# Sefaice/LearnRayTracing

Hardware: AMD Instinct MI355X
Metric: Mray/s at 1280×720, 4 spp, 8-bounce; 1/2/4/8-GPU scaling (higher is better)
Workload: dtype f32

## Files before the change

### learnraytracing_amd/csrc/lrt_diag.hip

```cpp
#include "lrt_grid_build.h"
#include "lrt_internal.h"

namespace lrt {

LRT_HD float libm_eval(int kind, float x) {
    if (kind == 6 || kind == 7) {
        float sn, cs;
        libm::sincosf(x, &sn, &cs);
        return kind == 6 ? sn : cs;
    }
    return kind == 0   ? libm::sinf(x)
           : kind == 1 ? libm::cosf(x)
           : kind == 2 ? libm::powf5(x)
           : kind == 3 ? libm::powf(x, 0.416666667f)
           : kind == 4 ? sqrt_rn(x)
                       : rcp_rn(x);
}

__global__ void libm_kernel(int kind, const float* __restrict__ in, float* __restrict__ out, long long n) {
    long long i = (long long)blockIdx.x * blockDim.x + threadIdx.x;
    if (i >= n) return;
    float x = in[i];
    out[i] = libm_eval(kind, x);
}


template <int kAcc>
LRT_DEV void scatter_case(const SceneView& sc, int i, const int* ids, const float* rays, const float* recs,
                          const uint32_t* seeds, float* out, int* ret, int* counted, uint32_t* state,
                          bool coherent = false) {
    const Ray r = make_ray(f3(rays[6 * i], rays[6 * i + 1], rays[6 * i + 2]),
                           f3(rays[6 * i + 3], rays[6 * i + 4], rays[6 * i + 5]));
    Hit rec;
// ... 357 lines not shown
        g.all = (const float4*)up(sph.data(), sizeof(float4) * sph.size());
        need.insert(need.end(), {(void*)g.cells, (void*)g.rsph, (void*)g.rid, (void*)g.bsph, (void*)g.bid, (void*)g.all});
    }
    auto release = [&]() {
        for (void* p : owned) (void)hipFree(p);
    };
    if (std::find(need.begin(), need.end(), nullptr) != need.end()) {
        release();
        return fail(LRT_E_NOMEM, "accel eval: device allocation failed");
    }
    const unsigned blocks = (unsigned)((n + 63) / 64);
    if (accel == 1) accel_probe_kernel<kAccBvh><<<blocks, 64>>>(bv, g, (const float*)d_rays, n, o_ids, o_ts, mode == 2);
    else accel_probe_kernel<kAccGrid><<<blocks, 64>>>(bv, g, (const float*)d_rays, n, o_ids, o_ts, 0);
    hipError_t e = hipGetLastError();
    if (e == hipSuccess) e = hipDeviceSynchronize();
    if (e == hipSuccess) e = hipMemcpy(ids, o_ids, sizeof(int) * (size_t)n, hipMemcpyDeviceToHost);
    if (e == hipSuccess) e = hipMemcpy(ts, o_ts, sizeof(float) * (size_t)n, hipMemcpyDeviceToHost);
    release();
    if (e != hipSuccess) return fail(LRT_E_HIP, std::string("accel eval: ") + hipGetErrorString(e));
    return LRT_OK;
}

int lrt_libm_eval_host(int kind, const float* in, float* out, long long n) {
    if (kind < 0 || kind > 7 || !in || !out || n < 0) return fail(LRT_E_INVALID, "invalid libm eval arguments");
    for (long long i = 0; i < n; ++i)
        out[i] = libm_eval(kind, in[i]);
    return LRT_OK;
}

int lrt_libm_eval_device(int kind, const float* d_in, float* d_out, long long n) {
    if (kind < 0 || kind > 7 || !d_in || !d_out || n < 0) return fail(LRT_E_INVALID, "invalid libm eval arguments");
    if (n == 0) return LRT_OK;
    libm_kernel<<<(unsigned)((n + 255) / 256), 256, 0, nullptr>>>(kind, d_in, d_out, n);
    LRT_HIP(hipGetLastError());
    LRT_HIP(hipDeviceSynchronize());
    return LRT_OK;
}


int lrt_kernel_timing(int on) {
    lrt::g_ktiming_on = on != 0;
    lrt::g_ktiming_used = 0;
    return LRT_OK;
}
int lrt_kernel_times(float* ms, int max_n, int* n) {
    if (!n || (max_n > 0 && !ms)) return lrt::fail(LRT_E_INVALID, "lrt_kernel_times: null output");
    int k = 0;
    for (size_t i = 0; i < lrt::g_ktiming_used && k < max_n; ++i) {
        auto& p = lrt::g_ktiming_ev[i];
        LRT_HIP(hipEventSynchronize(p.b));
        float t = 0.0f;
        LRT_HIP(hipEventElapsedTime(&t, p.a, p.b));
        ms[k++] = t;
    }
// ... 6 lines not shown
```

### learnraytracing_amd/csrc/lrt_internal.h

```cpp
#pragma once
#include <hip/hip_runtime.h>
#include <rccl/rccl.h>
#ifndef LRT_ROCTX
#define LRT_ROCTX 0
#endif
#if LRT_ROCTX
#include <rocprofiler-sdk-roctx/roctx.h>
#endif
#include <math.h>
#include <stdio.h>
#include <string.h>

#include <algorithm>
#include <climits>
#include <cmath>
#include <mutex>
#include <type_traits>
#include <string>
#include <vector>

#include "lrt.h"
#include "lrt_diag.h"
#include "lrt_trace.h"

#define LRT_VERSION_STRING "lrt-mi355x 0.4.0 gfx950"

namespace lrt {

constexpr int kBlock = 64;
constexpr int kBlockWavesX = kBlock == 256 ? 2 : 1;
constexpr int kBlockWavesY = kBlock / 64 / kBlockWavesX;
constexpr int WaveCols(int split) { return split <= 8 ? 8 : 64 / split; }
constexpr int kV0Queues = 16;
constexpr int kCtrStride = 64;

constexpr int kMaxDepthSupported = 64;

constexpr int kWavesPerEU = 4;
constexpr int kPoolSamples = 4096;

struct KernelArgs {
    CameraDev cam;
    const float4* sph;
    const float4* mats;
    const int* lights;
    int count, nlights;
    int width, height;
    int x0, xc, y0, rows;
    int rb, rp, rph;
    int frame0, frames, maxDepth;
    float4* out;
    unsigned long long* rays;
    BvhView bv;
    GridView gv;
    int bvh_stack_offset;
    int grid_lds_offset;
    float4* ovf;
    unsigned long long* wtrace;
    unsigned long long* tiles;
    int ndl;
    float4* feat[6];
    int featMax;
    int regenMin;
    int lateFetch;
    const float* lerp;
    float4* samp;
    float* colbuf;
    int poolSlots;
    int splitFrom;
    int split16;
    const int* perm;
    unsigned* tcost;
// ... 57 lines not shown
        void* d_tmp = nullptr;
        size_t tmp_bytes = 0;
        hipEvent_t ev_rec = nullptr;
        bool rec_done = false;
        int donor = -1;
        std::vector<std::pair<hipStream_t, hipEvent_t>> uses;
        unsigned long long tick = 0;
    };
    struct Scratch {
        hipStream_t s = nullptr;
        void* p = nullptr;
        size_t bytes = 0;
        unsigned long long tick = 0;
        hipEvent_t ev = nullptr;
    };
    static constexpr unsigned long long kScratchIdle = 64;
    static constexpr int kScratchSlots = 8;
    Scratch scratch[kScratchSlots];
    static constexpr int kOrderSlots = 8;
    TileOrder order[kOrderSlots];
    unsigned long long order_tick = 0;
    hipStream_t stream = nullptr;
    int count = 0, nlights = 0;
    float4* d_sph = nullptr;
    float4* d_mats = nullptr;
    int* d_lights = nullptr;
    std::vector<lrt_sphere> spheres;
    std::vector<lrt_material> mats;
    float4* d_bvh_nodes = nullptr;
    float4* d_bvh_lsph = nullptr;
    int* d_bvh_lid = nullptr;
    BvhView bvh{};
    int bvh_on = 0;
    bool bvh_built = false;
    int bvh_stack_levels = kBvhStackLevels;
    uint2* d_grid_cells = nullptr;
    float4* d_grid_rsph = nullptr;
    int* d_grid_rid = nullptr;
    float4* d_grid_bsph = nullptr;
    int* d_grid_bid = nullptr;
    GridView gv{};
    bool grid_pick = false;
    bool grid_ok = false;
    bool grid_built = false;

    float* d_frame = nullptr;
// ... 183 lines not shown
```

### learnraytracing_amd/csrc/lrt_pool.h

```cpp
#pragma once

namespace lrt {

enum : int { kPoolIdle = 0, kPoolTrace = 1, kPoolDone = 2, kPoolEnded = 3 };

template <int kPix>
struct PoolTile {
    static constexpr int X = kPix >= 128 ? 16 : kPix >= 32 ? 8 : kPix >= 8 ? 4 : kPix >= 2 ? 2 : 1;
    static constexpr int Y = kPix / X;
    static_assert(X * Y == kPix && kPix <= 256, "kPix: a power of two up to 256");
};

#if defined(__HIP_DEVICE_COMPILE__)
typedef const __attribute__((address_space(4))) KernelArgs* KArgPtr;
__device__ __forceinline__ KArgPtr opaque_args() {
    KArgPtr p = (KArgPtr)__builtin_amdgcn_kernarg_segment_ptr();
    asm volatile("" : "+s"(p));
    return p;
}
#else
typedef const KernelArgs* KArgPtr;
__device__ __forceinline__ KArgPtr opaque_args() { return nullptr; }
#endif

template <int kAcc, int kW>
__device__ __forceinline__ GridView pool_grid_view(float4* smem) {
    GridView g = opaque_args()->gv;
    {
        float4* b = reinterpret_cast<float4*>(reinterpret_cast<char*>(smem) + opaque_args()->bvh_stack_offset);
        g.bsph = b;
        g.bid = reinterpret_cast<const int*>(b + g.nbig);
    }
    if (kW > 1) {
        char* base = reinterpret_cast<char*>(smem) + opaque_args()->grid_lds_offset;
        const unsigned ncell = (unsigned)(g.nx * g.ny * g.nz), nref = g.cells_refs;
        g.rsph = reinterpret_cast<const float4*>(base);
        g.cells = reinterpret_cast<const uint2*>(base + 16 * nref);
        g.rid = reinterpret_cast<const int*>(base + 16 * nref + 8 * ncell);
    }
    return g;
}

constexpr int kPoolGridWaves = 16;
template <int kW>
constexpr int pool_stack_bytes() { return 64 * kTraceLdsLevels * (kW > 1 ? 14 : 16); }

template <int MAXD, bool kLds, int kAcc, int kPix, int kNS = 0, int kW = 1>
__global__ __launch_bounds__(64 * kW, kWavesPerEU) void pool_kernel(
    const KernelArgs a) {
    static_assert(kNS == 0 || (kLds && !kAcc), "a fixed sphere count is for the LDS linear scan");
    static_assert(kW == 1 || (kAcc == kAccGrid && !kLds), "multi-wave blocks: the grid instance");
    constexpr int kLv = kTraceLdsLevels;
    constexpr bool kPacked = kW > 1;
    extern __shared__ float4 smem[];
    const int lane = kW > 1 ? (int)(threadIdx.x & 63u) : (int)threadIdx.x;
    const int tid = threadIdx.x;
    const int wave = kW > 1 ? (int)(threadIdx.x >> 6) : 0;
    const int wid = (int)blockIdx.x * kW + wave;
    const int nwaves = (int)gridDim.x * kW;
    (void)nwaves;
    double* s_pow = reinterpret_cast<double*>(reinterpret_cast<char*>(smem) + kW * pool_stack_bytes<kW>());
    {
        const libm::PowTables g = libm::pow_tables();
        for (int i = tid; i < 16; i += 64 * kW) {
            s_pow[i] = g.invc[i];
            s_pow[16 + i] = g.logc[i];
        }
        for (int i = tid; i < 32; i += 64 * kW) reinterpret_cast<uint64_t*>(s_pow + 32)[i] = g.exp2[i];
    }
    constexpr int kLutBytes = kAcc ? 0 : kRenormBytes;
    float* s_lut = kAcc ? nullptr : reinterpret_cast<float*>(s_pow + 64);
    if (!kAcc) renorm_lut_fill(s_lut, lane, 64);
    float4* s_sph = reinterpret_cast<float4*>(reinterpret_cast<char*>(smem) + kW * pool_stack_bytes<kW>() +
// ... 147 lines not shown
                const unsigned long long waitM = __ballot(state == kPoolIdle || state == kPoolEnded);
                if (waitM && (__popcll(waitM) >= a.regenMin || __ballot(state == kPoolTrace) == 0)) {
                    if (state == kPoolEnded) {
                        sec_count(sc, kSecFold);
                        F3 T = carry;
                        for (int d = depth - 1; d >= 0; --d) {
                            const float4 s = get(d);
                            const float4 b = sc.mats[3 * __float_as_int(s.w) + 2];
                            T = f3(s.x, s.y, s.z) + f3(b.x, b.y, b.z) * T;
                        }
                        slots[3 * k] = T.x;
                        slots[3 * k + 1] = T.y;
                        slots[3 * k + 2] = T.z;
                        state = kPoolIdle;
                    }
                    const unsigned long long needM = waitM;
                    if (state == kPoolIdle) {
                        k = next + __popcll(needM & below);
                        state = kPoolDone;
                        if (k < N) {
                            const int j = k & ((1 << lgP) - 1), f = fr0 + (k >> lgP);
                            const int lx = tx0 + (j & ((1 << lgW) - 1)), ly = ty0 + (j >> lgW);
                            const KArgPtr pa = opaque_args();
                            if (lx < pa->xc && ly < pa->rows) {
                                sec_count(sc, kSecCamera);
                                const int x = pa->x0 + lx;
                                const int rb = pa->rb;
                                const int y = pa->y0 + (ly / rb) * rb * pa->rp + pa->rph * rb + ly % rb;
                                rng = PixelSeed((uint32_t)x, (uint32_t)y, (uint32_t)f);
                                const float u = ((float)x + RandomFloat01(rng)) * invWidth;
                                const float v = ((float)y + RandomFloat01(rng)) * invHeight;
                                const CameraDev cam = pa->cam;
                                r = GetRay(cam, u, v, rng, sc.rnlut);
                                depth = 0;
                                prevLambert = false;
                                pend = false;
                                state = kPoolTrace;
                            } else {
                                state = kPoolIdle;
                            }
                        }
                    }
                    next += __popcll(needM);
                    if constexpr (kLate) {
                        if (!asked && next >= N && fr0 + roundFrames >= fend) {
                            if (lane == 0) fetched = atomicAdd(ctr, 1ull);
                            asked = true;
                        }
                    }
                }
                const unsigned long long traceM = __ballot(state == kPoolTrace);
                if (traceM == 0) {
                    if (__ballot(state == kPoolIdle || state == kPoolEnded) == 0) break;
                    continue;
                }
// ... 6 lines not shown
                int nid = -1;
                float nt = 0.0f;
                bool shade = false, fin = false;
                F3 leaf = f3(0.0f, 0.0f, 0.0f);
                if (state == kPoolTrace) {
                    sec_count(sc, coherent ? kSecHit0 : kSecHit);
                    ++rays;
                    bool lit = false;
                    const bool hasS = pend && dl.on;
                    if constexpr (kAcc == kAccGrid) {
                        const float4 ls = hasS ? sc.sph[dl.li] : make_float4(0.0f, 0.0f, 0.0f, 0.0f);
                        const GridView gv = pool_grid_view<kAcc, kW>(smem);
                        nid = ClosestHitDualGrid<(kW > 1 ? 1 : 0)>(r.orig, r.dir, hasS, dl.l, dl.li, ls, gv, nt, lit);
                    } else if constexpr (kAcc == kAccBvh) {
                        if (coherent) {
                            nid = ClosestHitBVH(r.orig, r.dir, sc.bv, nt, sc.bstk, sc.bstride, nullptr, true);
                        } else {
                            const float4 ls = hasS ? sc.sph[dl.li] : make_float4(0.0f, 0.0f, 0.0f, 0.0f);
                            nid = ClosestHitDualBVH4(r.orig, r.dir, hasS, dl.l, dl.li, ls, sc.bv, nt, lit, sc.bstk,
                                                     sc.bstride);
                        }
                    } else {
                        int sid;
                        DualClosestHit<kNS>(r.orig, r.dir, hasS, dl.l, sc, nid, nt, sid);
                        lit = hasS && sid == dl.li;
                    }
                    if (pend) {
                        if (lit) put(depth, make_float4(carry.x, carry.y, carry.z, __int_as_float(dl.id)));
                        ++depth;
                        pend = false;
                    }
                    if (nid < 0) {
                        const float t = 0.5f * (r.dir.y + 1.0f);
                        leaf = ((1.0f - t) * f3(1.0f, 1.0f, 1.0f) + t * f3(0.5f, 0.7f, 1.0f)) * 0.3f;
                        fin = true;
                    } else {
                        shade = true;
                    }
                }
                if (shade) {
                    const float4 sp4 = sc.sph[nid];
                    Hit rec;
                    rec.pos = point_at(r, nt);
                    rec.normal = normalize(rec.pos - f3(sp4.x, sp4.y, sp4.z));
                    rec.t = nt;
                    const Material mat = load_material(sc.mats, nid);
                    F3 matE = mat.emissive;
                    fin = true;
                    leaf = matE;
                    if (depth < a.maxDepth) {
                        F3 lightE;
                        dl.on = false;
                        if constexpr (kAcc == kAccGrid) sc.gv = pool_grid_view<kAcc, kW>(smem);
                        const F3 X = ScatterDir<kAcc, kNS>(mat, nid, r, rec, lightE, rays, rng, sc, &dl, coherent);
                        sec_count(sc, kSecPost);
                        const F3 dir = renormalize(normalize(X), sc.rnlut);
                        if ((mat.type != 1) | (dot(dir, rec.normal) > 0.0f)) {
                            if (a.ndl && prevLambert) matE = f3(0.0f, 0.0f, 0.0f);
                            prevLambert = mat.type == 0;
                            const F3 e = matE + lightE;
                            put(depth, make_float4(e.x, e.y, e.z, __int_as_float(nid)));
                            if (dl.on) carry = matE + (lightE + dl.contrib);
                            dl.id = nid;
                            pend = true;
                            r.orig = rec.pos;
                            r.dir = dir;
                            fin = false;
                        }
                    }
                }
                if (fin) {
                    carry = leaf;
                    state = kPoolEnded;
                }
            }
            sec_enter(sc, kSecOther, false);
            __builtin_amdgcn_fence(__ATOMIC_RELEASE, "workgroup");
// ... 16 lines not shown
                        float lf[4];
#pragma unroll
                        for (int u = 0; u < 4; ++u) {
                            const float* const cp = slots + 3 * (((t + u) << lgP) + j);
                            c[u] = f3(cp[0], cp[1], cp[2]);
                            const int f = fr0 + t + u;
                            lf[u] = f < kLerpTable ? lerp[f] : (float)f / (float)(f + 1);
                        }
#pragma unroll
                        for (int u = 0; u < 4; ++u) c3 = c3 * lf[u] + c[u] * (1.0f - lf[u]);
                    }
                    for (; t < nfr; ++t) {
                        const float* const cp = slots + 3 * ((t << lgP) + j);
                        const F3 c = f3(cp[0], cp[1], cp[2]);
                        const int f = fr0 + t;
                        const float lerpFac = f < kLerpTable ? lerp[f] : (float)f / (float)(f + 1);
                        c3 = c3 * lerpFac + f3(c.x, c.y, c.z) * (1.0f - lerpFac);
                    }
                    acc.x = c3.x;
                    acc.y = c3.y;
                    acc.z = c3.z;
                    *mpx = acc;
                    if (frame) {
                        const int rb = pa->rb;
                        const int gy = pa->y0 + (my / rb) * rb * pa->rp + pa->rph * rb + my % rb;
                        frame[(size_t)gy * pa->width + pa->x0 + mx] = acc;
                    }
                }
            }
            __builtin_amdgcn_fence(__ATOMIC_RELEASE, "workgroup");
            __builtin_amdgcn_fence(__ATOMIC_ACQUIRE, "workgroup");
        }
        if (a.tcost && lane == 0) a.tcost[tile] = (unsigned)(__builtin_amdgcn_s_memrealtime() - tt0);
        if constexpr (kLate)
            if (!asked && lane == 0) fetched = atomicAdd(ctr, 1ull);
        const unsigned long long n = __shfl(fetched, 0, 64) + (unsigned long long)bq;
        i = n < (unsigned long long)nq ? (int)n : nq;
    }
#ifdef LRT_EXP_SECSTATS
    sec_enter(sc, kSecOther, false);
    if (lane == 0)
        for (int k = 0; k < kSecN; ++k) {
            unsigned long long* g = sc.secstats + 3 * (k + kSecN * (wid & 15));
            atomicAdd(g, sc.sectime[2 + kSecN + k]);
            atomicAdd(g + 1, sc.sectime[2 + 2 * kSecN + k]);
            atomicAdd(g + 2, sc.sectime[2 + k]);
        }
#endif
// ... 20 lines not shown
```

### learnraytracing_amd/csrc/lrt_pool_launch.h

```cpp
#pragma once
#include "lrt_internal.h"
#include "lrt_pool.h"

namespace lrt {

inline int pool_grid_wpb(const KernelArgs& a, size_t stack_w, size_t shared_b, size_t static_b, size_t* grid_b) {
    const size_t ncell = (size_t)a.gv.nx * a.gv.ny * a.gv.nz, nref = a.gv.cells_refs;
    *grid_b = (16 * nref + 8 * ncell + 4 * nref + 15) / 16 * 16;
    if (!a.gv.on || a.gv.nx == 0) return 1;
    int dev = 0, maxb = 0;
    if (hipGetDevice(&dev) != hipSuccess ||
        hipDeviceGetAttribute(&maxb, hipDeviceAttributeMaxSharedMemoryPerBlock, dev) != hipSuccess)
        return 1;
    return kPoolGridWaves * stack_w + shared_b + *grid_b + static_b <= (size_t)maxb ? kPoolGridWaves : 1;
}

template <int MAXD, int kPix>
int launch_pool(KernelArgs a, bool lds, int xc, int rows, hipStream_t s) {
    constexpr int TX = PoolTile<kPix>::X, TY = PoolTile<kPix>::Y;
    constexpr int kW = kPoolGridWaves;
    const long long ntiles = (long long)((xc + TX - 1) / TX) * ((rows + TY - 1) / TY);
    const int acc = a.gv.on ? kAccGrid : a.bv.on ? kAccBvh : kAccScan;
    const size_t bstk = acc == kAccBvh ? sizeof(unsigned short) * ctx().bvh_stack_levels * 64
                        : acc == kAccGrid ? (sizeof(float4) + sizeof(int)) * (size_t)a.gv.nbig : 0;
// ... 8 lines not shown
                  ? pool_grid_wpb(a, pool_stack_bytes<kW>(), kPowTableBytes + (bstk + 15) / 16 * 16, static_b, &grid_b)
                  : 1;
    if (wpb > 1) {
        static signed char raised[kMaxDevices * 4] = {};
        int dev = 0, maxb = 0;
        signed char* r = hipGetDevice(&dev) == hipSuccess && dev >= 0 && dev < kMaxDevices * 4 ? &raised[dev] : nullptr;
        if (r && *r == 0)
            *r = hipDeviceGetAttribute(&maxb, hipDeviceAttributeMaxSharedMemoryPerBlock, dev) == hipSuccess &&
                         hipFuncSetAttribute((const void*)pool_kernel<MAXD, false, kAccGrid, kPix, 0, kW>,
                                             hipFuncAttributeMaxDynamicSharedMemorySize,
                                             maxb - (int)static_b) == hipSuccess
                     ? 1
                     : -1;
        if (!r || *r < 0) wpb = 1;
    }
    const int lv = kTraceLdsLevels;
    const size_t stack = (wpb > 1 ? (size_t)pool_stack_bytes<kW>() * wpb : (size_t)pool_stack_bytes<1>()) +
                         kPowTableBytes + (acc ? 0 : kRenormBytes);
    const size_t scene = lds ? sizeof(float4) * (4 * (size_t)a.count + (size_t)(a.nlights + 3) / 4 + 1) : 0;
    a.bvh_stack_offset = (int)(stack + scene);
    a.grid_lds_offset = wpb > 1 ? (int)(stack + (bstk + 15) / 16 * 16) : 0;
    const size_t ldsb = wpb > 1 ? stack + (bstk + 15) / 16 * 16 + grid_b : stack + scene + bstk;
    const bool fixed = lds && acc == kAccScan && a.count == kFixedSpheres;
    const void* kern = acc == kAccGrid ? (lds ? (const void*)pool_kernel<MAXD, true, kAccGrid, kPix>
                                          : wpb > 1 ? (const void*)pool_kernel<MAXD, false, kAccGrid, kPix, 0, kW>
                                              : (const void*)pool_kernel<MAXD, false, kAccGrid, kPix>)
                       : acc == kAccBvh ? (lds ? (const void*)pool_kernel<MAXD, true, kAccBvh, kPix>
                                               : (const void*)pool_kernel<MAXD, false, kAccBvh, kPix>)
                       : (fixed ? (const void*)pool_kernel<MAXD, true, kAccScan, kPix, kFixedSpheres>
                          : lds ? (const void*)pool_kernel<MAXD, true, kAccScan, kPix>
                                : (const void*)pool_kernel<MAXD, false, kAccScan, kPix>);
    int per_cu = 0;
    hipError_t e = occupancy(&per_cu, kern, 64 * wpb, ldsb);
    if (e != hipSuccess) return hip_fail(e, "hipOccupancyMaxActiveBlocksPerMultiprocessor");
    if (per_cu < 1) return fail(LRT_E_INVALID, "pool_kernel does not fit on a CU");
    int cus = ctx().num_cus;
    for (const auto& m : ctx().masked_streams)
        if (m.first == s) cus = m.second;
    long long blocks = std::max((long long)per_cu * cus, (long long)kV0Queues);
    if (blocks > ntiles) blocks = ntiles;
    const dim3 grid((unsigned)blocks);
    a.ovf = nullptr;
    a.colbuf = nullptr;
    a.tiles = ctx().d_tiles + (size_t)(ctx().tiles_next++ % kQueueSlots) * kTileSetU64;
    a.regenMin = 16;
    a.lateFetch = ntiles < 6LL * (long long)grid.x * wpb ? 1 : 0;
    a.poolSlots = kPix * std::min(a.frames, kPoolSamples / kPix);
// ... 23 lines not shown
    a.splitFrom = split ? (int)(ntiles - ntiles * a.split16 / 16) : (int)ntiles;
    bool probed = false;
    if (record == 1 && pool_probe_mode() > 0 && (pool_probe_mode() == 2 || !users[1])) {
        Context::TileOrder& o = *users[0];
        KernelArgs pa = a;
        pa.bvh_stack_offset = 0;
        e = launch_tile_probe(pa, acc, o, (int)ntiles, TX, TY, bstk, s);
        if (e != hipSuccess) {
            o.state = 0;
            return hip_fail(e, "tile cost probe");
        }
        a.perm = o.d_perm;
        users[1] = nullptr;
        probed = true;
    }
    kernel_timing(s, 0);
    if (acc == kAccGrid) {
        if (lds) pool_kernel<MAXD, true, kAccGrid, kPix><<<grid, 64, ldsb, s>>>(a);
        else if (wpb > 1) pool_kernel<MAXD, false, kAccGrid, kPix, 0, kW><<<grid, 64 * kW, ldsb, s>>>(a);
        else pool_kernel<MAXD, false, kAccGrid, kPix><<<grid, 64, ldsb, s>>>(a);
    } else if (acc == kAccBvh) {
        if (lds) pool_kernel<MAXD, true, kAccBvh, kPix><<<grid, 64, ldsb, s>>>(a);
        else pool_kernel<MAXD, false, kAccBvh, kPix><<<grid, 64, ldsb, s>>>(a);
    } else if (fixed) {
        pool_kernel<MAXD, true, kAccScan, kPix, kFixedSpheres><<<grid, 64, ldsb, s>>>(a);
    } else {
        if (lds) pool_kernel<MAXD, true, kAccScan, kPix><<<grid, 64, ldsb, s>>>(a);
        else pool_kernel<MAXD, false, kAccScan, kPix><<<grid, 64, ldsb, s>>>(a);
    }
    kernel_timing(s, 1);
    e = hipGetLastError();
    if (e != hipSuccess) {
        if (record) users[0]->state = 0;
        return hip_fail(e, "pool_kernel launch");
    }
    e = stream_scratch_used(s);
    if (e != hipSuccess) return hip_fail(e, "pool scratch event");
    if (record) {
        Context::TileOrder& o = *users[0];
        e = sort_tiles_desc(o.d_cost, o.d_keys, o.d_ids, o.d_sort_out, (int)ntiles, o.d_tmp, &o.tmp_bytes, s);
        if (e == hipSuccess) e = hipEventRecord(o.ev_rec, s);
        if (e != hipSuccess) {
            o.state = 0;
            return hip_fail(e, "tile order sort");
        }
    }
    for (auto* u : users)
        if (u)
            if (int rc = order_used(*u, s)) return rc;
    snprintf(g_last_launch, sizeof(g_last_launch),
             "kernel=pool_kernel maxd=%d lds=%d bvh=%d acc=%s pix=%d ns=%d grid=%u tasks=%lld order=%d per_cu=%d wpb=%d "
             "split_from=%d",
             MAXD, lds ? 1 : 0, acc == kAccBvh ? 1 : 0, acc_name(acc), kPix, fixed ? kFixedSpheres : 0, grid.x, ntiles,
             !users[0] ? 0 : !record ? 2 : record == 2 ? 5 : probed ? 4 : users[1] ? 3 : 1, per_cu, wpb, a.splitFrom);
#ifdef LRT_EXP_SECSTATS
    secstats_dump(d_sec, s);
#endif
#ifdef LRT_EXP_WAVETRACE
    wavetrace_dump(a.wtrace, grid.x, s);
#endif
    return LRT_OK;
}

template <int MAXD>
int launch_pool_split(const KernelArgs& a, bool lds, int xc, int rows, int frames, int pix_cap, hipStream_t s) {
    switch (pool_pixels(frames, xc, rows, pix_cap)) {
        case 256: return launch_pool<MAXD, 256>(a, lds, xc, rows, s);
        case 128: return launch_pool<MAXD, 128>(a, lds, xc, rows, s);
        case 64: return launch_pool<MAXD, 64>(a, lds, xc, rows, s);
        case 32: return launch_pool<MAXD, 32>(a, lds, xc, rows, s);
        case 16: return launch_pool<MAXD, 16>(a, lds, xc, rows, s);
        case 4: return launch_pool<MAXD, 4>(a, lds, xc, rows, s);
        default: return launch_pool<MAXD, 1>(a, lds, xc, rows, s);
    }
}

}
// ... 1 lines not shown
```

### learnraytracing_amd/csrc/lrt_render.hip

```cpp
#include "lrt_internal.h"

namespace lrt {

__global__ void merge_samples_kernel(const float4* __restrict__ samp, float4* __restrict__ out, const float* lerp,
                                     int npix, int frame0, int frames, size_t stride, const KernelArgs a, int pix0) {
    const int i = blockIdx.x * blockDim.x + threadIdx.x;
    if (i >= npix) return;
    const float4 o = out[i];
    F3 acc = f3(o.x, o.y, o.z);
    for (int k = 0; k < frames; ++k) {
        const float4 c = samp[(size_t)k * stride + i];
        const int f = frame0 + k;
        const float lerpFac = f < kLerpTable ? lerp[f] : (float)f / (float)(f + 1);
        acc = acc * lerpFac + f3(c.x, c.y, c.z) * (1.0f - lerpFac);
    }
    float* d = reinterpret_cast<float*>(out + i);
    d[0] = acc.x;
    d[1] = acc.y;
    d[2] = acc.z;
    if (a.frame) {
        const int p = pix0 + i, lx = p % a.xc, ly = p / a.xc;
        a.frame[(size_t)GlobalRow(a, ly) * a.width + a.x0 + lx] = make_float4(acc.x, acc.y, acc.z, o.w);
    }
}
// ... 310 lines not shown
    const lrt_camera& c = d->camera;
    a.cam.origin = f3(c.origin.x, c.origin.y, c.origin.z);
    a.cam.a = f3(c.a.x, c.a.y, c.a.z);
    a.cam.u = f3(c.u.x, c.u.y, c.u.z);
    a.cam.r = f3(c.r.x, c.r.y, c.r.z);
    a.cam.llc = f3(c.lowerLeftCorner.x, c.lowerLeftCorner.y, c.lowerLeftCorner.z);
    a.cam.horiz = f3(c.horizontalVec.x, c.horizontalVec.y, c.horizontalVec.z);
    a.cam.vert = f3(c.verticalVec.x, c.verticalVec.y, c.verticalVec.z);
    a.cam.lensRadius = c.lensRadius;
    a.sph = ctx().d_sph;
    a.mats = ctx().d_mats;
    a.lights = ctx().d_lights;
    a.count = ctx().count;
    a.nlights = ctx().nlights;
    a.width = d->width;
    a.height = d->height;
    a.x0 = d->x0;
    a.xc = d->x_count;
    a.y0 = d->y0;
    a.rows = d->row_count;
    a.rb = d->row_block;
    a.rp = d->row_period;
    a.rph = d->row_phase;
    a.frame0 = d->frame0;
    a.frames = d->frames;
    a.maxDepth = d->max_depth;
    a.out = reinterpret_cast<float4*>(d_buf);
    a.rays = d_rays;
    a.ndl = (d->flags & LRT_F_NO_DOUBLE_LIGHT) ? 1 : 0;
    bool want_feat = false;
    {
        float* const fp[6] = {feat ? feat->normal : nullptr,    feat ? feat->world_pos : nullptr,
                              feat ? feat->albedo : nullptr,    feat ? feat->color_std : nullptr,
                              feat ? feat->normal_std : nullptr, feat ? feat->world_pos_std : nullptr};
        for (int k = 0; k < 6; ++k) {
            a.feat[k] = reinterpret_cast<float4*>(fp[k]);
            want_feat = want_feat || fp[k] != nullptr;
        }
        a.featMax = feat ? feat->max_frame : -1;
    }
    const bool use_grid = ctx().grid_ok && !(d->flags & LRT_F_NO_BVH) && !want_feat && !(d->flags & LRT_F_BVH) &&
                          (ctx().grid_pick || (d->flags & LRT_F_GRID));
    const bool use_bvh = ctx().bvh_on && !(d->flags & LRT_F_NO_BVH) && !use_grid;
    if (use_grid)
        if (int rc = ensure_grid(ctx())) return rc;
    if (use_bvh)
// ... 63 lines not shown
```

### learnraytracing_amd/csrc/lrt_scene.hip

```cpp
#include <functional>

#include "lrt_grid_build.h"
#include "lrt_internal.h"

namespace lrt {

const lrt_sphere kDefaultSpheres[9] = {
    {{0, -100.5f, -1}, 100.0f}, {{2, 1, -1}, 0.5f},  {{0, 0, -1}, 0.5f},
    {{-2, 0, -1}, 0.5f},        {{2, 0, 1}, 0.5f},   {{0, 0, 1}, 0.5f},
    {{-2, 0, 1}, 0.5f},         {{0.5f, 1, 0.5f}, 0.5f}, {{-1.5f, 1.5f, 0.f}, 0.3f},
};
const lrt_material kDefaultMats[9] = {
    {LRT_LAMBERT, {0.8f, 0.8f, 0.8f}, {0, 0, 0}, 0, 0},
    {LRT_LAMBERT, {0.8f, 0.4f, 0.4f}, {0, 0, 0}, 0, 0},
    {LRT_LAMBERT, {0.4f, 0.8f, 0.4f}, {0, 0, 0}, 0, 0},
    {LRT_METAL, {0.4f, 0.4f, 0.8f}, {0, 0, 0}, 0, 0},
    {LRT_METAL, {0.4f, 0.8f, 0.4f}, {0, 0, 0}, 0, 0},
    {LRT_METAL, {0.4f, 0.8f, 0.4f}, {0, 0, 0}, 0.2f, 0},
    {LRT_METAL, {0.4f, 0.8f, 0.4f}, {0, 0, 0}, 0.6f, 0},
    {LRT_DIELECTRIC, {0.4f, 0.4f, 0.4f}, {0, 0, 0}, 0, 1.5f},
    {LRT_LAMBERT, {0.8f, 0.6f, 0.2f}, {30, 25, 15}, 0, 0},
};

constexpr int kBvhLeaf = 6;
// ... 396 lines not shown
        build_grid_host(s, n, sph, G);
        have_grid = true;
        pick = accel ? grid_suitable(G) : true;
    }
    const bool have_bvh = accel && !pick;
    if (have_bvh) {
        build_bvh_host(s, n, sph, B);
        if (B.stack_levels > kBvhStackLevels) return fail(LRT_E_INVALID, "BVH deeper than the traversal stack");
    }
    free_scene(c);
    LRT_HIP(upload(c.d_sph, sph));
    LRT_HIP(upload(c.d_mats, mats));
    LRT_HIP(upload(c.d_lights, lights));
    c.bvh_on = accel ? 1 : 0;
    c.grid_ok = n > 0;
    c.grid_pick = pick;
    if (have_bvh)
        if (int rc = upload_bvh(c, B)) return rc;
    if (have_grid)
        if (int rc = upload_grid(c, G)) return rc;
    c.count = n;
    ++c.scene_version;
    c.nlights = (int)lights.size();
    c.spheres.assign(s, s + n);
    c.mats.assign(m, m + n);
    return LRT_OK;
}

lrt_float3 L3(float x, float y, float z) {
    lrt_float3 r = {x, y, z};
    return r;
}
lrt_float3 h_sub(lrt_float3 a, lrt_float3 b) { return L3(a.x - b.x, a.y - b.y, a.z - b.z); }
lrt_float3 h_smul(float a, lrt_float3 b) { return L3(a * b.x, a * b.y, a * b.z); }
lrt_float3 h_cross(lrt_float3 a, lrt_float3 b) {
    return L3(a.y * b.z - a.z * b.y, -(a.x * b.z - a.z * b.x), a.x * b.y - a.y * b.x);
}
lrt_float3 h_normalize(lrt_float3 v) {
    float k = 1.0f / sqrtf(v.x * v.x + v.y * v.y + v.z * v.z);
    return L3(v.x * k, v.y * k, v.z * k);
}

int camera_make(lrt_float3 lookFrom, lrt_float3 lookAt, lrt_float3 vup, float vfov, float aspect, float aperture,
                float focusDist, lrt_camera* out) {
    if (!out) return fail(LRT_E_INVALID, "camera out is NULL");
    lrt_camera c;
// ... 24 lines not shown
```

### learnraytracing_amd/csrc/lrt_trace.h

```cpp
#pragma once
#include <hip/hip_runtime.h>
#include <stdint.h>

#include "lrt_libm.h"

namespace lrt {

#define LRT_DEV __host__ __device__ __forceinline__

constexpr float kPI = 3.1415926f;
constexpr float kMinT = 0.001f;
constexpr float kMaxT = 1.0e7f;

struct float3_ { float x, y, z; };
using F3 = float3_;

LRT_DEV F3 f3(float x, float y, float z) { F3 r; r.x = x; r.y = y; r.z = z; return r; }
LRT_DEV F3 operator+(F3 a, F3 b) { return f3(a.x + b.x, a.y + b.y, a.z + b.z); }
LRT_DEV F3 operator-(F3 a, F3 b) { return f3(a.x - b.x, a.y - b.y, a.z - b.z); }
LRT_DEV F3 operator*(F3 a, F3 b) { return f3(a.x * b.x, a.y * b.y, a.z * b.z); }
LRT_DEV F3 operator*(F3 a, float b) { return f3(a.x * b, a.y * b, a.z * b); }
LRT_DEV F3 operator*(float a, F3 b) { return f3(a * b.x, a * b.y, a * b.z); }
LRT_DEV F3 operator-(F3 a) { return f3(-a.x, -a.y, -a.z); }
LRT_DEV float dot(F3 a, F3 b) { return a.x * b.x + a.y * b.y + a.z * b.z; }
LRT_DEV F3 cross(F3 a, F3 b) {
    return f3(a.y * b.z - a.z * b.y, -(a.x * b.z - a.z * b.x), a.x * b.y - a.y * b.x);
}
LRT_DEV float sqrt_rn(float x) {
#if defined(__HIP_DEVICE_COMPILE__)
    float s = __builtin_amdgcn_sqrtf(x);
    const float sd = __int_as_float(__float_as_int(s) - 1);
    const float su = __int_as_float(__float_as_int(s) + 1);
    const float rd = __builtin_fmaf(-sd, s, x);
    const float ru = __builtin_fmaf(-su, s, x);
    s = rd <= 0.0f ? sd : s;
    s = ru > 0.0f ? su : s;
    if (__builtin_expect(__ballot(!(x >= 0x1p-96f)) != 0, 0)) s = __builtin_sqrtf(x);
    return s;
#else
    return __builtin_sqrtf(x);
#endif
}
LRT_DEV float rcp_rn(float x) {
#if defined(__HIP_DEVICE_COMPILE__)
    float r = __builtin_amdgcn_rcpf(x);
    float e = __builtin_fmaf(-x, r, 1.0f);
    r = __builtin_fmaf(e, r, r);
    e = __builtin_fmaf(-x, r, 1.0f);
    r = __builtin_fmaf(e, r, r);
    const float ax = __builtin_fabsf(x);
    if (__builtin_expect(__ballot(!(ax >= 0x1p-125f && ax <= 0x1p125f)) != 0, 0)) r = 1.0f / x;
    return r;
#else
    return 1.0f / x;
#endif
}
LRT_DEV float length(F3 v) { return sqrt_rn(v.x * v.x + v.y * v.y + v.z * v.z); }
LRT_DEV F3 normalize(F3 v) { float k = rcp_rn(length(v)); return f3(v.x * k, v.y * k, v.z * k); }
constexpr int kRenormR = 64;
constexpr int kRenormBytes = ((2 * kRenormR + 1) * 4 + 15) / 16 * 16;
LRT_DEV void renorm_lut_fill(float* lut, int tid, int block) {
    for (int j = tid; j <= 2 * kRenormR; j += block) {
        const float d = libm::u2f((uint32_t)(0x3f800000 + j - kRenormR));
        lut[j] = rcp_rn(sqrt_rn(d));
    }
}
constexpr int kPowTableBytes = 16 * 8 + 16 * 8 + 32 * 8;
LRT_DEV F3 normalize_member(F3 v) { float l = length(v); return f3(v.x / l, v.y / l, v.z / l); }
LRT_DEV F3 reflect(F3 v, F3 n) { return v + 2.0f * (-dot(v, n) * n); }
LRT_DEV bool refract(F3 v, F3 n, float nint, F3& out) {
    float dt = dot(v, n);
    float discr = 1.0f - nint * nint * (1.0f - dt * dt);
    if (discr > 0) {
        out = nint * (v - n * dt) - n * sqrt_rn(discr);
        return true;
    }
    return false;
}
LRT_DEV float schlick(float cosine, float ri, const libm::PowTables& T) {
    float r0 = (1.0f - ri) / (1.0f + ri);
    r0 = r0 * r0;
// ... 111 lines not shown
LRT_DEV void sec_enter(const SceneView& sc, int sec, bool count) {
#if defined(LRT_EXP_SECSTATS) && defined(__HIP_DEVICE_COMPILE__)
    const unsigned long long m = __ballot(1);
    if ((int)__lane_id() == __ffsll((long long)m) - 1) {
        const unsigned long long now = __builtin_amdgcn_s_memtime();
        unsigned long long* w = sc.sectime;
        const int cur = (int)w[0];
        w[2 + cur] += now - w[1];
        w[0] = (unsigned long long)sec;
        w[1] = now;
        if (count) {
            w[2 + kSecN + sec] += 1;
            w[2 + 2 * kSecN + sec] += (unsigned long long)__popcll(m);
        }
    }
#else
    (void)sc;
    (void)sec;
    (void)count;
#endif
}
LRT_DEV void sec_count(const SceneView& sc, int sec) { sec_enter(sc, sec, true); }

LRT_DEV void SphereRoots(float rsProj, float ifHit, float tMin, float& closestT, int& id, int i) {
    if (ifHit < 0.0f) {
        const float halfCut = sqrt_rn(-ifHit);
        const float t1 = rsProj - halfCut, t2 = rsProj + halfCut;
        const bool ok1 = (t1 > tMin) & (t1 < closestT);
        const bool ok2 = (t2 > tMin) & (t2 < closestT);
        id = (ok1 | ok2) ? i : id;
        closestT = ok1 ? t1 : ok2 ? t2 : closestT;
    }
}

template <int kAcc = 0, int kNS = 0>
LRT_DEV int ClosestHitSV(const Ray& r, float tMin, float tMax, const SceneView& sc, float& tOut,
                         bool coherent = false) {
    if constexpr (kAcc == kAccGrid)
        return ClosestHitGrid(r.orig, r.dir, sc.gv, tOut);
    if constexpr (kAcc == kAccBvh)
        return ClosestHitBVH(r.orig, r.dir, sc.bv, tOut, sc.bstk, sc.bstride, nullptr, coherent);
    float closestT = tMax;
    int id = -1;
    auto test = [&](int i, const float4& s) {
        F3 rs = f3(s.x, s.y, s.z) - r.orig;
        float rsProj = dot(rs, r.dir);
        float ifHit = dot(rs, rs) - rsProj * rsProj - s.w;
        SphereRoots(rsProj, ifHit, tMin, closestT, id, i);
    };
// ... 32 lines not shown

template <int kAcc = 0, int kNS = 0>
LRT_DEV bool HitWorld(const Ray& r, float tMin, float tMax, const SceneView& sc, Hit& outHit, int& outID,
                      bool coherent = false) {
    float closestT;
    sec_count(sc, coherent ? kSecHit0 : kSecHit);
    const int id = ClosestHitSV<kAcc, kNS>(r, tMin, tMax, sc, closestT, coherent);
    if (id < 0) return false;
    float4 s = sc.sph[id];
    outHit.pos = point_at(r, closestT);
    outHit.normal = normalize(outHit.pos - f3(s.x, s.y, s.z));
    outHit.t = closestT;
    outID = id;
    return true;
}

struct DeferredLight {
    F3 l, contrib;
    int li;
    bool on;
    int id;
};

template <int kAcc = 0, int kNS = 0>
LRT_DEV F3 ScatterDir(const Material& mat, int matId, const Ray& r_in, const Hit& rec, F3& outLightE,
                      int& inoutRayCount, uint32_t& rng, const SceneView& sc, DeferredLight* defer = nullptr,
                      bool coherent = false) {
    outLightE = f3(0.0f, 0.0f, 0.0f);
    if (mat.type == 0) {
        sec_count(sc, kSecLambert);
        const int i0 = sc.nlights > 0 ? sc.lights[0] : 0;
        const float4 s0 = sc.sph[i0];
        F3 target = rec.pos + rec.normal + RandomUnitVector(rng);
        const F3 X = target - rec.pos;
        for (int k = 0; k < sc.nlights; ++k) {
            int i = k == 0 ? i0 : sc.lights[k];
            if (i == matId) continue;
            float4 s = k == 0 ? s0 : sc.sph[i];
            F3 c = f3(s.x, s.y, s.z);
            const F3 cp = c - rec.pos;
            const float len = length(cp);
            const float kinv = rcp_rn(len);
            F3 sw = f3(cp.x * kinv, cp.y * kinv, cp.z * kinv);
            F3 su = normalize(cross(__builtin_fabsf(sw.x) > 0.01f ? f3(0.0f, 1.0f, 0.0f) : f3(1.0f, 0.0f, 0.0f), sw));
            F3 sv = cross(sw, su);
            float cosAMax = sqrt_rn(1.0f - s.w / (len * len));
            float eps1 = RandomFloat01(rng);
            float eps2 = RandomFloat01(rng);
            float cosA = 1.0f - eps1 + eps1 * cosAMax;
            float sinA = sqrt_rn(1.0f - cosA * cosA);
            float phi = 2.0f * kPI * eps2;
            float sphi, cphi;
            libm::sincosf(phi, &sphi, &cphi);
            F3 l = su * cphi * sinA + sv * sphi * sinA + sw * cosA;
            l = normalize_member(l);
            float tLight;
            ++inoutRayCount;
            if (defer && k == sc.nlights - 1) {
                float omega = 2.0f * kPI * (1.0f - cosAMax);
                F3 rdir = r_in.dir;
                F3 nl = dot(rec.normal, rdir) < 0.0f ? rec.normal : -rec.normal;
                float d = dot(l, nl);
                float mx = (0.0f < d) ? d : 0.0f;
                const float4 e = sc.mats[3 * i + 1];
                defer->l = renormalize(l, sc.rnlut);
                defer->contrib = (mat.albedo * f3(e.x, e.y, e.z)) * (mx * omega / kPI);
                defer->li = i;
                defer->on = true;
                continue;
            }
            sec_count(sc, coherent ? kSecShadow0 : kSecShadow);
            bool lit;
            if constexpr (kAcc == kAccGrid) {
                lit = ShadowReachesLightGrid(rec.pos, renormalize(l, sc.rnlut), i, s, sc.gv);
            } else if constexpr (kAcc == kAccBvh) {
                Ray sr;
                sr.orig = rec.pos;
                sr.dir = renormalize(l, sc.rnlut);
                lit = ShadowReachesLightBVH(sr.orig, sr.dir, i, s, sc.bv, sc.bstk, sc.bstride, coherent);
            } else {
                Ray sr;
// ... 97 lines not shown
            sec_count(sc, kSecPost);
            if (ndl && prevLambert) matE = f3(0.0f, 0.0f, 0.0f);
            prevLambert = mat.type == 0;
            F3 e = matE + lightE;
            put(depth, make_float4(e.x, e.y, e.z, __int_as_float(id)));
            ++depth;
            r = scattered;
            continue;
        }
        leaf = matE;
        break;
    }
    F3 T = leaf;
    sec_count(sc, kSecFold);
    for (int d = depth - 1; d >= 0; --d) {
        float4 s = get(d);
        float4 b = sc.mats[3 * __float_as_int(s.w) + 2];
        T = f3(s.x, s.y, s.z) + f3(b.x, b.y, b.z) * T;
    }
    sec_enter(sc, kSecOther, false);
    return T;
}

template <int kNS = 0>
LRT_DEV void DualClosestHit(const F3& o, const F3& db, bool hasShadow, const F3& ds, const SceneView& sc,
                            int& idB, float& tB, int& idS) {
    float closestB = kMaxT, closestS = kMaxT;
    idB = -1;
    idS = -1;
    auto test = [&](int i, const float4& s) {
        const F3 rs = f3(s.x, s.y, s.z) - o;
        const float rr = dot(rs, rs);
        {
            const float rsProj = dot(rs, db);
            const float ifHit = rr - rsProj * rsProj - s.w;
            SphereRoots(rsProj, ifHit, kMinT, closestB, idB, i);
        }
        if (hasShadow) {
            const float rsProj = dot(rs, ds);
            const float ifHit = rr - rsProj * rsProj - s.w;
            SphereRoots(rsProj, ifHit, kMinT, closestS, idS, i);
        }
    };
    if constexpr (kNS > 0) {
        float4 next = sc.sph[0];
#pragma unroll
        for (int i = 0; i < kNS; ++i) {
            const float4 s = next;
            if (i + 1 < kNS) next = sc.sph[i + 1];
            test(i, s);
        }
    } else {
        float4 next = sc.sph[0];
        for (int i = 0; i < sc.count; ++i) {
            const float4 s = next;
            if (i + 1 < sc.count) next = sc.sph[i + 1];
            test(i, s);
        }
    }
    tB = closestB;
}

template <int MAXD, bool kFeat = false, int kLdsLev = kTraceLdsLevels, int kNS = 0>
LRT_DEV F3 TraceDual(Ray r, int maxDepth, int& inoutRayCount, uint32_t& rng, const SceneView& sc,
// ... 93 lines not shown
```

Baseline: 58380.

## Add trimmed fixed-scene kernel variant skipping range checks and specializing light count

Splits sqrt/rcp into fast and range-checked versions and uses the unchecked sqrt in sphere root solving. The unchecked path is only taken by a new pool kernel instance selected when the fixed scene has one light and every sphere radius² is above a threshold verified on the host. It also fuses normalize into a single rsqrt-length helper with one combined ballot check, and adds a rowIdent flag that skips the row-interleave arithmetic when the row period is 1. Together these remove per-call wave ballots and integer div/mod in hot loops. The cost is an extra kernel template instance and more reliance on host-side invariants.

```diff
diff --git a/learnraytracing_amd/csrc/lrt_diag.hip b/learnraytracing_amd/csrc/lrt_diag.hip
--- a/learnraytracing_amd/csrc/lrt_diag.hip
+++ b/learnraytracing_amd/csrc/lrt_diag.hip
@@ -9,6 +9,9 @@
         libm::sincosf(x, &sn, &cs);
         return kind == 6 ? sn : cs;
     }
+    if (kind == 8) return rsqrt_len(x);
+    if (kind == 9) return rcp_rn(sqrt_rn(x));
+    if (kind == 10) return sqrt_fast(x);
     return kind == 0   ? libm::sinf(x)
            : kind == 1 ? libm::cosf(x)
            : kind == 2 ? libm::powf5(x)
@@ -412,14 +415,14 @@
 }
 
 int lrt_libm_eval_host(int kind, const float* in, float* out, long long n) {
-    if (kind < 0 || kind > 7 || !in || !out || n < 0) return fail(LRT_E_INVALID, "invalid libm eval arguments");
+    if (kind < 0 || kind > 10 || !in || !out || n < 0) return fail(LRT_E_INVALID, "invalid libm eval arguments");
     for (long long i = 0; i < n; ++i)
         out[i] = libm_eval(kind, in[i]);
     return LRT_OK;
 }
 
 int lrt_libm_eval_device(int kind, const float* d_in, float* d_out, long long n) {
-    if (kind < 0 || kind > 7 || !d_in || !d_out || n < 0) return fail(LRT_E_INVALID, "invalid libm eval arguments");
+    if (kind < 0 || kind > 10 || !d_in || !d_out || n < 0) return fail(LRT_E_INVALID, "invalid libm eval arguments");
     if (n == 0) return LRT_OK;
     libm_kernel<<<(unsigned)((n + 255) / 256), 256, 0, nullptr>>>(kind, d_in, d_out, n);
     LRT_HIP(hipGetLastError());
diff --git a/learnraytracing_amd/csrc/lrt_internal.h b/learnraytracing_amd/csrc/lrt_internal.h
--- a/learnraytracing_amd/csrc/lrt_internal.h
+++ b/learnraytracing_amd/csrc/lrt_internal.h
@@ -41,13 +41,14 @@
 
 struct KernelArgs {
     CameraDev cam;
+    int x0, xc, y0, rows;
+    int rb, rp, rph;
+    int rowIdent;
     const float4* sph;
     const float4* mats;
     const int* lights;
     int count, nlights;
     int width, height;
-    int x0, xc, y0, rows;
-    int rb, rp, rph;
     int frame0, frames, maxDepth;
     float4* out;
     unsigned long long* rays;
@@ -151,6 +152,7 @@
     unsigned long long order_tick = 0;
     hipStream_t stream = nullptr;
     int count = 0, nlights = 0;
+    bool roots_in_range = false;
     float4* d_sph = nullptr;
     float4* d_mats = nullptr;
     int* d_lights = nullptr;
diff --git a/learnraytracing_amd/csrc/lrt_pool.h b/learnraytracing_amd/csrc/lrt_pool.h
--- a/learnraytracing_amd/csrc/lrt_pool.h
+++ b/learnraytracing_amd/csrc/lrt_pool.h
@@ -45,10 +45,11 @@
 template <int kW>
 constexpr int pool_stack_bytes() { return 64 * kTraceLdsLevels * (kW > 1 ? 14 : 16); }
 
-template <int MAXD, bool kLds, int kAcc, int kPix, int kNS = 0, int kW = 1>
+template <int MAXD, bool kLds, int kAcc, int kPix, int kNS = 0, int kW = 1, int kNL = 0, bool kChk = true>
 __global__ __launch_bounds__(64 * kW, kWavesPerEU) void pool_kernel(
     const KernelArgs a) {
     static_assert(kNS == 0 || (kLds && !kAcc), "a fixed sphere count is for the LDS linear scan");
+    static_assert((kNL == 0 && kChk) || kNS > 0, "a fixed light count and unchecked roots: fixed-scene instances");
     static_assert(kW == 1 || (kAcc == kAccGrid && !kLds), "multi-wave blocks: the grid instance");
     constexpr int kLv = kTraceLdsLevels;
     constexpr bool kPacked = kW > 1;
@@ -242,15 +243,17 @@
                             const int j = k & ((1 << lgP) - 1), f = fr0 + (k >> lgP);
                             const int lx = tx0 + (j & ((1 << lgW) - 1)), ly = ty0 + (j >> lgW);
                             const KArgPtr pa = opaque_args();
-                            if (lx < pa->xc && ly < pa->rows) {
+                            const int wx0 = pa->x0, wxc = pa->xc, wy0 = pa->y0, wrows = pa->rows;
+                            const int rb = pa->rb, rp = pa->rp, rph = pa->rph, rowIdent = pa->rowIdent;
+                            const CameraDev cam = pa->cam;
+                            if (lx < wxc && ly < wrows) {
                                 sec_count(sc, kSecCamera);
-                                const int x = pa->x0 + lx;
-                                const int rb = pa->rb;
-                                const int y = pa->y0 + (ly / rb) * rb * pa->rp + pa->rph * rb + ly % rb;
+                                const int x = wx0 + lx;
+                                int y = wy0 + ly;
+                                if (!rowIdent) y = wy0 + (ly / rb) * rb * rp + rph * rb + ly % rb;
                                 rng = PixelSeed((uint32_t)x, (uint32_t)y, (uint32_t)f);
                                 const float u = ((float)x + RandomFloat01(rng)) * invWidth;
                                 const float v = ((float)y + RandomFloat01(rng)) * invHeight;
-                                const CameraDev cam = pa->cam;
                                 r = GetRay(cam, u, v, rng, sc.rnlut);
                                 depth = 0;
                                 prevLambert = false;
@@ -303,7 +306,7 @@
                         }
                     } else {
                         int sid;
-                        DualClosestHit<kNS>(r.orig, r.dir, hasS, dl.l, sc, nid, nt, sid);
+                        DualClosestHit<kNS, kChk>(r.orig, r.dir, hasS, dl.l, sc, nid, nt, sid);
                         lit = hasS && sid == dl.li;
                     }
                     if (pend) {
@@ -333,7 +336,7 @@
                         F3 lightE;
                         dl.on = false;
                         if constexpr (kAcc == kAccGrid) sc.gv = pool_grid_view<kAcc, kW>(smem);
-                        const F3 X = ScatterDir<kAcc, kNS>(mat, nid, r, rec, lightE, rays, rng, sc, &dl, coherent);
+                        const F3 X = ScatterDir<kAcc, kNS, kNL>(mat, nid, r, rec, lightE, rays, rng, sc, &dl, coherent);
                         sec_count(sc, kSecPost);
                         const F3 dir = renormalize(normalize(X), sc.rnlut);
                         if ((mat.type != 1) | (dot(dir, rec.normal) > 0.0f)) {
@@ -396,8 +399,11 @@
                     acc.z = c3.z;
                     *mpx = acc;
                     if (frame) {
-                        const int rb = pa->rb;
-                        const int gy = pa->y0 + (my / rb) * rb * pa->rp + pa->rph * rb + my % rb;
+                        int gy = pa->y0 + my;
+                        if (!pa->rowIdent) {
+                            const int rb = pa->rb;
+                            gy = pa->y0 + (my / rb) * rb * pa->rp + pa->rph * rb + my % rb;
+                        }
                         frame[(size_t)gy * pa->width + pa->x0 + mx] = acc;
                     }
                 }
diff --git a/learnraytracing_amd/csrc/lrt_pool_launch.h b/learnraytracing_amd/csrc/lrt_pool_launch.h
--- a/learnraytracing_amd/csrc/lrt_pool_launch.h
+++ b/learnraytracing_amd/csrc/lrt_pool_launch.h
@@ -54,7 +54,11 @@
     a.grid_lds_offset = wpb > 1 ? (int)(stack + (bstk + 15) / 16 * 16) : 0;
     const size_t ldsb = wpb > 1 ? stack + (bstk + 15) / 16 * 16 + grid_b : stack + scene + bstk;
     const bool fixed = lds && acc == kAccScan && a.count == kFixedSpheres;
-    const void* kern = acc == kAccGrid ? (lds ? (const void*)pool_kernel<MAXD, true, kAccGrid, kPix>
+    constexpr bool kTrimmed = MAXD <= 8;
+    const bool trim = kTrimmed && fixed && a.nlights == 1 && ctx().roots_in_range;
+    const void* kern_trim = nullptr;
+    if constexpr (kTrimmed) kern_trim = (const void*)pool_kernel<MAXD, true, kAccScan, kPix, kFixedSpheres, 1, 1, false>;
+    const void* kern = trim ? kern_trim : acc == kAccGrid ? (lds ? (const void*)pool_kernel<MAXD, true, kAccGrid, kPix>
                                           : wpb > 1 ? (const void*)pool_kernel<MAXD, false, kAccGrid, kPix, 0, kW>
                                               : (const void*)pool_kernel<MAXD, false, kAccGrid, kPix>)
                        : acc == kAccBvh ? (lds ? (const void*)pool_kernel<MAXD, true, kAccBvh, kPix>
@@ -124,6 +128,8 @@
     } else if (acc == kAccBvh) {
         if (lds) pool_kernel<MAXD, true, kAccBvh, kPix><<<grid, 64, ldsb, s>>>(a);
         else pool_kernel<MAXD, false, kAccBvh, kPix><<<grid, 64, ldsb, s>>>(a);
+    } else if (trim) {
+        if constexpr (kTrimmed) pool_kernel<MAXD, true, kAccScan, kPix, kFixedSpheres, 1, 1, false><<<grid, 64, ldsb, s>>>(a);
     } else if (fixed) {
         pool_kernel<MAXD, true, kAccScan, kPix, kFixedSpheres><<<grid, 64, ldsb, s>>>(a);
     } else {
@@ -152,9 +158,9 @@
             if (int rc = order_used(*u, s)) return rc;
     snprintf(g_last_launch, sizeof(g_last_launch),
              "kernel=pool_kernel maxd=%d lds=%d bvh=%d acc=%s pix=%d ns=%d grid=%u tasks=%lld order=%d per_cu=%d wpb=%d "
-             "split_from=%d",
+             "split_from=%d chk=%d nl=%d",
              MAXD, lds ? 1 : 0, acc == kAccBvh ? 1 : 0, acc_name(acc), kPix, fixed ? kFixedSpheres : 0, grid.x, ntiles,
-             !users[0] ? 0 : !record ? 2 : record == 2 ? 5 : probed ? 4 : users[1] ? 3 : 1, per_cu, wpb, a.splitFrom);
+             !users[0] ? 0 : !record ? 2 : record == 2 ? 5 : probed ? 4 : users[1] ? 3 : 1, per_cu, wpb, a.splitFrom, trim ? 0 : 1, trim ? 1 : 0);
 #ifdef LRT_EXP_SECSTATS
     secstats_dump(d_sec, s);
 #endif
diff --git a/learnraytracing_amd/csrc/lrt_render.hip b/learnraytracing_amd/csrc/lrt_render.hip
--- a/learnraytracing_amd/csrc/lrt_render.hip
+++ b/learnraytracing_amd/csrc/lrt_render.hip
@@ -356,6 +356,7 @@
     a.rb = d->row_block;
     a.rp = d->row_period;
     a.rph = d->row_phase;
+    a.rowIdent = d->row_period == 1 ? 1 : 0;
     a.frame0 = d->frame0;
     a.frames = d->frames;
     a.maxDepth = d->max_depth;
diff --git a/learnraytracing_amd/csrc/lrt_scene.hip b/learnraytracing_amd/csrc/lrt_scene.hip
--- a/learnraytracing_amd/csrc/lrt_scene.hip
+++ b/learnraytracing_amd/csrc/lrt_scene.hip
@@ -442,6 +442,8 @@
     c.count = n;
     ++c.scene_version;
     c.nlights = (int)lights.size();
+    c.roots_in_range = true;
+    for (const float4& q : sph) c.roots_in_range = c.roots_in_range && q.w >= 0x1p-70f;
     c.spheres.assign(s, s + n);
     c.mats.assign(m, m + n);
     return LRT_OK;
diff --git a/learnraytracing_amd/csrc/lrt_trace.h b/learnraytracing_amd/csrc/lrt_trace.h
--- a/learnraytracing_amd/csrc/lrt_trace.h
+++ b/learnraytracing_amd/csrc/lrt_trace.h
@@ -26,7 +26,7 @@
 LRT_DEV F3 cross(F3 a, F3 b) {
     return f3(a.y * b.z - a.z * b.y, -(a.x * b.z - a.z * b.x), a.x * b.y - a.y * b.x);
 }
-LRT_DEV float sqrt_rn(float x) {
+LRT_DEV float sqrt_fast(float x) {
 #if defined(__HIP_DEVICE_COMPILE__)
     float s = __builtin_amdgcn_sqrtf(x);
     const float sd = __int_as_float(__float_as_int(s) - 1);
@@ -35,28 +35,53 @@
     const float ru = __builtin_fmaf(-su, s, x);
     s = rd <= 0.0f ? sd : s;
     s = ru > 0.0f ? su : s;
-    if (__builtin_expect(__ballot(!(x >= 0x1p-96f)) != 0, 0)) s = __builtin_sqrtf(x);
     return s;
 #else
     return __builtin_sqrtf(x);
 #endif
 }
-LRT_DEV float rcp_rn(float x) {
+LRT_DEV float rcp_fast(float x) {
 #if defined(__HIP_DEVICE_COMPILE__)
     float r = __builtin_amdgcn_rcpf(x);
     float e = __builtin_fmaf(-x, r, 1.0f);
     r = __builtin_fmaf(e, r, r);
     e = __builtin_fmaf(-x, r, 1.0f);
     r = __builtin_fmaf(e, r, r);
-    const float ax = __builtin_fabsf(x);
-    if (__builtin_expect(__ballot(!(ax >= 0x1p-125f && ax <= 0x1p125f)) != 0, 0)) r = 1.0f / x;
     return r;
 #else
     return 1.0f / x;
 #endif
 }
+LRT_DEV float sqrt_rn(float x) {
+    float s = sqrt_fast(x);
+#if defined(__HIP_DEVICE_COMPILE__)
+    if (__builtin_expect(__ballot(!(x >= 0x1p-96f)) != 0, 0)) s = __builtin_sqrtf(x);
+#endif
+    return s;
+}
+LRT_DEV float rcp_rn(float x) {
+    float r = rcp_fast(x);
+#if defined(__HIP_DEVICE_COMPILE__)
+    const float ax = __builtin_fabsf(x);
+    if (__builtin_expect(__ballot(!(ax >= 0x1p-125f && ax <= 0x1p125f)) != 0, 0)) r = 1.0f / x;
+#endif
+    return r;
+}
 LRT_DEV float length(F3 v) { return sqrt_rn(v.x * v.x + v.y * v.y + v.z * v.z); }
-LRT_DEV F3 normalize(F3 v) { float k = rcp_rn(length(v)); return f3(v.x * k, v.y * k, v.z * k); }
+LRT_DEV float rsqrt_len(float d) {
+#if defined(__HIP_DEVICE_COMPILE__)
+    float k = rcp_fast(sqrt_fast(d));
+    if (__builtin_expect(__ballot(libm::f2u(d) - 0x0f800000u > 0x7f7fffffu - 0x0f800000u) != 0, 0))
+        k = rcp_rn(sqrt_rn(d));
+    return k;
+#else
+    return 1.0f / __builtin_sqrtf(d);
+#endif
+}
+LRT_DEV F3 normalize(F3 v) {
+    float k = rsqrt_len(v.x * v.x + v.y * v.y + v.z * v.z);
+    return f3(v.x * k, v.y * k, v.z * k);
+}
 constexpr int kRenormR = 64;
 constexpr int kRenormBytes = ((2 * kRenormR + 1) * 4 + 15) / 16 * 16;
 LRT_DEV void renorm_lut_fill(float* lut, int tid, int block) {
@@ -214,9 +239,10 @@
 }
 LRT_DEV void sec_count(const SceneView& sc, int sec) { sec_enter(sc, sec, true); }
 
+template <bool kChk = true>
 LRT_DEV void SphereRoots(float rsProj, float ifHit, float tMin, float& closestT, int& id, int i) {
     if (ifHit < 0.0f) {
-        const float halfCut = sqrt_rn(-ifHit);
+        const float halfCut = kChk ? sqrt_rn(-ifHit) : sqrt_fast(-ifHit);
         const float t1 = rsProj - halfCut, t2 = rsProj + halfCut;
         const bool ok1 = (t1 > tMin) & (t1 < closestT);
         const bool ok2 = (t2 > tMin) & (t2 < closestT);
@@ -295,18 +321,19 @@
     int id;
 };
 
-template <int kAcc = 0, int kNS = 0>
+template <int kAcc = 0, int kNS = 0, int kNL = 0>
 LRT_DEV F3 ScatterDir(const Material& mat, int matId, const Ray& r_in, const Hit& rec, F3& outLightE,
                       int& inoutRayCount, uint32_t& rng, const SceneView& sc, DeferredLight* defer = nullptr,
                       bool coherent = false) {
     outLightE = f3(0.0f, 0.0f, 0.0f);
     if (mat.type == 0) {
         sec_count(sc, kSecLambert);
-        const int i0 = sc.nlights > 0 ? sc.lights[0] : 0;
+        const int nlights = kNL > 0 ? kNL : sc.nlights;
+        const int i0 = nlights > 0 ? sc.lights[0] : 0;
         const float4 s0 = sc.sph[i0];
         F3 target = rec.pos + rec.normal + RandomUnitVector(rng);
         const F3 X = target - rec.pos;
-        for (int k = 0; k < sc.nlights; ++k) {
+        for (int k = 0; k < nlights; ++k) {
             int i = k == 0 ? i0 : sc.lights[k];
             if (i == matId) continue;
             float4 s = k == 0 ? s0 : sc.sph[i];
@@ -329,7 +356,7 @@
             l = normalize_member(l);
             float tLight;
             ++inoutRayCount;
-            if (defer && k == sc.nlights - 1) {
+            if (defer && k == nlights - 1) {
                 float omega = 2.0f * kPI * (1.0f - cosAMax);
                 F3 rdir = r_in.dir;
                 F3 nl = dot(rec.normal, rdir) < 0.0f ? rec.normal : -rec.normal;
@@ -473,7 +500,7 @@
     return T;
 }
 
-template <int kNS = 0>
+template <int kNS = 0, bool kChk = true>
 LRT_DEV void DualClosestHit(const F3& o, const F3& db, bool hasShadow, const F3& ds, const SceneView& sc,
                             int& idB, float& tB, int& idS) {
     float closestB = kMaxT, closestS = kMaxT;
@@ -485,12 +512,12 @@
         {
             const float rsProj = dot(rs, db);
             const float ifHit = rr - rsProj * rsProj - s.w;
-            SphereRoots(rsProj, ifHit, kMinT, closestB, idB, i);
+            SphereRoots<kChk>(rsProj, ifHit, kMinT, closestB, idB, i);
         }
         if (hasShadow) {
             const float rsProj = dot(rs, ds);
             const float ifHit = rr - rsProj * rsProj - s.w;
-            SphereRoots(rsProj, ifHit, kMinT, closestS, idS, i);
+            SphereRoots<kChk>(rsProj, ifHit, kMinT, closestS, idS, i);
         }
     };
     if constexpr (kNS > 0) {
```

Measured after the change: 60910 (median of 6 runs). 1.04x the previous value.
